# chrischoy/DeepGlobalRegistration

Measured on NVIDIA H100. Metric: scan_pairs_per_sec, higher is better.
Workload: dtype f32

## Files before the change

deepglobalregistration_b200/csrc/knn_tc.cu:

```cuda
#include <algorithm>

#include "common.cuh"
#include "tc_common.cuh"

namespace {

using namespace tc;

constexpr int kRows = 128;
constexpr int kTileBytes = kRows * 128;
constexpr int kTileFloats = kTileBytes / 4;
constexpr int kConsumerWarps = 8;
constexpr int kThreads = kConsumerWarps * 32 + 128;
constexpr int kQueue = 256;
constexpr float kInf = __builtin_huge_valf();

template <int C>
struct KnnCfg {
  static constexpr int kChunks = C / 32;
  static constexpr int kStages = C == 32 ? 4 : 3;
  static constexpr int kOpBytes = kChunks * kTileBytes;
  static constexpr size_t kSmem = 1024 + (size_t)(2 + kStages) * kOpBytes + kStages * kRows * 4 +
                                  kConsumerWarps * (kQueue + 16) * 8 + (2 * kStages + 4) * 8 + 16;
};

struct KnnWs {
  float* a_img;
  float* b_img;
  float* na2;
  unsigned* rowmin;
  float* nbh;
  float* bmax;
};
inline int64_t up4(int64_t x) { return (x + 3) & ~(int64_t)3; }
inline int64_t ceil_tiles(int64_t n) { return (n + kRows - 1) / kRows; }
void ws_offsets(int64_t n0, int64_t n1, int c, int64_t (&o)[7]) {
  const int64_t tile = (int64_t)(c / 32) * kTileFloats;
  o[0] = 0;
  o[1] = o[0] + ceil_tiles(n0) * tile;
  o[2] = o[1] + ceil_tiles(n1) * tile;
  o[3] = o[2] + up4(n0);
  o[4] = o[3] + up4(n0);
  o[5] = o[4] + ceil_tiles(n1) * kRows;
  o[6] = o[5] + up4(ceil_tiles(n1));
}
KnnWs carve_ws(float* ws, int64_t n0, int64_t n1, int c) {
  int64_t o[7];
  ws_offsets(n0, n1, c, o);
  return KnnWs{ws + o[0], ws + o[1], ws + o[2], reinterpret_cast<unsigned*>(ws + o[3]), ws + o[4], ws + o[5]};
}

__device__ __forceinline__ float knn_error_bound(float na, float nb) {
  return (0.0009765625f * 1.25f + 4e-5f) * na * nb + 1e-6f * (na + nb) * (na + nb) + 1e-7f;
}

template <int C>
__global__ void __launch_bounds__(kRows * 8)
knn_prep_kernel(const float* __restrict__ f0, int n0, const float* __restrict__ f1, int n1, int row_tiles, KnnWs w,
                unsigned long long* __restrict__ packed) {
  constexpr int kChunks = C / 32;
  const bool is_a = (int)blockIdx.x < row_tiles;
  const int tile = is_a ? blockIdx.x : blockIdx.x - row_tiles;
  const float* f = is_a ? f0 : f1;
  const int n = is_a ? n0 : n1;
  const int r = threadIdx.x >> 3, sub = threadIdx.x & 7;
  const int row = tile * kRows + r;
  const bool valid = row < n;
  float s = 0.f;
  if (valid)
    for (int k = sub; k < C; k += 8) {
      const float v = f[(size_t)row * C + k];
      s = fmaf(v, v, s);
    }
  s += __shfl_xor_sync(0xffffffffu, s, 1);
  s += __shfl_xor_sync(0xffffffffu, s, 2);
  s += __shfl_xor_sync(0xffffffffu, s, 4);
  float* img = (is_a ? w.a_img : w.b_img) + (size_t)tile * kChunks * kTileFloats;
#pragma unroll
  for (int ch = 0; ch < kChunks; ++ch) {
    float4 v = make_float4(0.f, 0.f, 0.f, 0.f);
    if (valid) v = __ldg(reinterpret_cast<const float4*>(f + (size_t)row * C + ch * 32 + sub * 4));
    v.x = tf32_round(v.x); v.y = tf32_round(v.y); v.z = tf32_round(v.z); v.w = tf32_round(v.w);
    *reinterpret_cast<float4*>(img + ch * kTileFloats + r * 32 + ((sub ^ (r & 7)) << 2)) = v;
  }
  if (is_a) {
    if (valid && sub == 0) {
      w.na2[row] = s;
      w.rowmin[row] = 0x7f800000u;
      packed[row] = ~0ull;
    }
    return;
  }
  if (sub == 0) w.nbh[row] = valid ? 0.5f * s : kInf;
  __shared__ float wmax[kRows * 8 / 32];
  float m = valid ? s : 0.f;
  m = fmaxf(m, __shfl_xor_sync(0xffffffffu, m, 8));
  m = fmaxf(m, __shfl_xor_sync(0xffffffffu, m, 16));
  if ((threadIdx.x & 31) == 0) wmax[threadIdx.x >> 5] = m;
  __syncthreads();
  if (threadIdx.x < 32) {
    m = wmax[threadIdx.x];
#pragma unroll
    for (int d = 16; d > 0; d >>= 1) m = fmaxf(m, __shfl_xor_sync(0xffffffffu, m, d));
    if (threadIdx.x == 0) w.bmax[tile] = m;
  }
}

template <int C>
__device__ __forceinline__ unsigned long long knn_exact_key(const float* __restrict__ f0, const float* __restrict__ f1,
                                                            int gi, int j) {
  const float4* a = reinterpret_cast<const float4*>(f0 + (size_t)gi * C);
  const float4* b = reinterpret_cast<const float4*>(f1 + (size_t)j * C);
  float d2 = 0.f;
#pragma unroll
  for (int k = 0; k < C / 4; ++k) {
    const float4 x = __ldg(a + k), y = __ldg(b + k);
    float df = x.x - y.x; d2 = fmaf(df, df, d2);
    df = x.y - y.y; d2 = fmaf(df, df, d2);
    df = x.z - y.z; d2 = fmaf(df, df, d2);
    df = x.w - y.w; d2 = fmaf(df, df, d2);
  }
  return ((unsigned long long)__float_as_uint(sqrtf(d2 + 1e-7f)) << 32) | (unsigned)j;
}

struct Item {
  int rt, ct0, ct1;
};
__device__ __forceinline__ Item item_at(long long k, long long k_end, int col_tiles) {
  Item it;
  it.rt = (int)(k / col_tiles);
  it.ct0 = (int)(k - (long long)it.rt * col_tiles);
  it.ct1 = (int)min((long long)col_tiles, it.ct0 + (k_end - k));
  return it;
}

template <int C, int PASS>
__global__ void __launch_bounds__(kThreads, 1)
knn_sweep_kernel(const float* __restrict__ f0, int n0, const float* __restrict__ f1, int row_tiles, int col_tiles,
                 KnnWs w, unsigned long long* __restrict__ packed) {
  using K = KnnCfg<C>;
  constexpr int kStages = K::kStages, kOpBytes = K::kOpBytes;
  extern __shared__ __align__(16) unsigned char smem_dyn[];
  unsigned char* a_buf = reinterpret_cast<unsigned char*>((reinterpret_cast<uintptr_t>(smem_dyn) + 1023) &
                                                          ~(uintptr_t)1023);
  unsigned char* b_buf = a_buf + 2 * kOpBytes;
  float* nb_buf = reinterpret_cast<float*>(b_buf + kStages * kOpBytes);
  unsigned long long* queue = reinterpret_cast<unsigned long long*>(nb_buf + kStages * kRows);
  unsigned long long* best = queue + kConsumerWarps * kQueue;
  uint64_t* bars = reinterpret_cast<uint64_t*>(best + kConsumerWarps * 16);
  const uint32_t full0 = smem_u32(bars), empty0 = full0 + 8 * kStages;
  const uint32_t a_full0 = empty0 + 8 * kStages, a_empty0 = a_full0 + 16;
  float* nbmax_sh = reinterpret_cast<float*>(bars + 2 * kStages + 4);

  const int t = threadIdx.x, warp = __shfl_sync(0xffffffffu, t >> 5, 0), lane = t & 31;
  const long long total = (long long)row_tiles * col_tiles;
  const long long k_begin = total * blockIdx.x / gridDim.x, k_end = total * (blockIdx.x + 1) / gridDim.x;

  if (t == 0) {
    for (int s = 0; s < kStages; ++s) {
      mbar_init(full0 + 8 * s, 1);
      mbar_init(empty0 + 8 * s, kConsumerWarps);
    }
    for (int p = 0; p < 2; ++p) {
      mbar_init(a_full0 + 8 * p, 1);
      mbar_init(a_empty0 + 8 * p, kConsumerWarps);
    }
    asm volatile("fence.mbarrier_init.release.cluster;" ::: "memory");
  }
  if (PASS == 2 && warp == 0) {
    float m = 0.f;
    for (int i = lane; i < col_tiles; i += 32) m = fmaxf(m, w.bmax[i]);
#pragma unroll
    for (int d = 16; d > 0; d >>= 1) m = fmaxf(m, __shfl_xor_sync(0xffffffffu, m, d));
    if (lane == 0) *nbmax_sh = m;
  }
  if (PASS == 2 && t < kConsumerWarps * 16) best[t] = ~0ull;
  __syncthreads();

  if (warp >= kConsumerWarps) {
    asm volatile("setmaxnreg.dec.sync.aligned.u32 40;");
    if (warp == kConsumerWarps && lane == 0) {
      long long kt = 0;
      int it = 0;
      for (long long k = k_begin; k < k_end; ++it) {
        const Item item = item_at(k, k_end, col_tiles);
        const int p = it & 1;
        if (it >= 2) mbar_wait(a_empty0 + 8 * p, ((it >> 1) - 1) & 1);
        mbar_arrive_expect_tx(a_full0 + 8 * p, kOpBytes);
        bulk_g2s(smem_u32(a_buf + p * kOpBytes), w.a_img + (size_t)item.rt * (kOpBytes / 4), kOpBytes, a_full0 + 8 * p);
        for (int ct = item.ct0; ct < item.ct1; ++ct, ++kt) {
          const int s = (int)(kt % kStages);
          if (kt >= kStages) mbar_wait(empty0 + 8 * s, (uint32_t)((kt / kStages - 1) & 1));
          mbar_arrive_expect_tx(full0 + 8 * s, kOpBytes + kRows * 4);
          bulk_g2s(smem_u32(b_buf + s * kOpBytes), w.b_img + (size_t)ct * (kOpBytes / 4), kOpBytes, full0 + 8 * s);
          bulk_g2s(smem_u32(nb_buf + s * kRows), w.nbh + (size_t)ct * kRows, kRows * 4, full0 + 8 * s);
        }
        k += item.ct1 - item.ct0;
      }
    }
    return;
  }

  asm volatile("setmaxnreg.inc.sync.aligned.u32 232;");
  const int wg = warp >> 2;
  const int rw = lane >> 2;
  const int row_in_tile = wg * 64 + (warp & 3) * 16;
  const float nb_root = PASS == 2 ? sqrtf(*nbmax_sh) : 0.f;
  unsigned long long* q = queue + warp * kQueue;
  unsigned long long* bw = best + warp * 16;
  int qn = 0;

  auto drain = [&](int row0) {
    __syncwarp();
    for (int b = 0; b < qn; b += 32)
      if (b + lane < qn) {
        const unsigned long long e = q[b + lane];
        const int r = (int)(e >> 32), j = (int)(unsigned)e;
        atomicMin(bw + r, knn_exact_key<C>(f0, f1, row0 + r, j));
      }
    qn = 0;
    __syncwarp();
  };

  long long kt = 0;
  int it = 0;
  for (long long k = k_begin; k < k_end; ++it) {
    const Item item = item_at(k, k_end, col_tiles);
    const int p = it & 1;
    const int row0 = item.rt * kRows + row_in_tile;
    int gi[2];
    float th[2], rmin[2][2];
#pragma unroll
    for (int h = 0; h < 2; ++h) {
      gi[h] = row0 + rw + 8 * h;
      th[h] = -kInf;
      if (PASS == 2 && gi[h] < n0) {
        const float na2 = w.na2[gi[h]];
        const float e = knn_error_bound(sqrtf(na2), nb_root);
        th[h] = 0.5f * (__uint_as_float(w.rowmin[gi[h]]) + 4.f * e - na2);
      }
      rmin[h][0] = rmin[h][1] = kInf;
    }
    mbar_wait(a_full0 + 8 * p, (it >> 1) & 1);
    const uint32_t a_s = smem_u32(a_buf + p * kOpBytes) + wg * (kTileBytes / 2);

    auto issue = [&](float(&acc)[64], long long kq) {
      const int s = (int)(kq % kStages);
      mbar_wait(full0 + 8 * s, (uint32_t)((kq / kStages) & 1));
      const uint32_t b_s = smem_u32(b_buf + s * kOpBytes);
      wgmma_fence();
#pragma unroll
      for (int ch = 0; ch < K::kChunks; ++ch)
#pragma unroll
        for (int ks = 0; ks < 4; ++ks)
          Wgmma<128, false>::mma(acc, wgmma_desc(a_s + ch * kTileBytes + ks * 32),
                                 wgmma_desc(b_s + ch * kTileBytes + ks * 32), (ch | ks) != 0);
      wgmma_commit();
    };
    auto epilogue = [&](float(&acc)[64], long long kq, int ct) {
      fence_acc(acc);
      const int s = (int)(kq % kStages);
      const float* nbs = nb_buf + s * kRows + 2 * (lane & 3);
      float tmin[2][2] = {{kInf, kInf}, {kInf, kInf}};
#pragma unroll
      for (int i = 0; i < kRows / 8; ++i) {
        const float2 nb = *reinterpret_cast<const float2*>(nbs + 8 * i);
#pragma unroll
        for (int h = 0; h < 2; ++h)
          tmin[h][i & 1] = fminf(tmin[h][i & 1], fminf(nb.x - acc[4 * i + 2 * h], nb.y - acc[4 * i + 2 * h + 1]));
      }
      if (PASS == 1) {
#pragma unroll
        for (int h = 0; h < 2; ++h) {
          rmin[h][0] = fminf(rmin[h][0], tmin[h][0]);
          rmin[h][1] = fminf(rmin[h][1], tmin[h][1]);
        }
      } else if (__any_sync(0xffffffffu, fminf(tmin[0][0], tmin[0][1]) <= th[0] ||
                                             fminf(tmin[1][0], tmin[1][1]) <= th[1])) {
        unsigned long long mask = 0;
#pragma unroll
        for (int i = 0; i < kRows / 8; ++i) {
          const float2 nb = *reinterpret_cast<const float2*>(nbs + 8 * i);
#pragma unroll
          for (int h = 0; h < 2; ++h)
#pragma unroll
            for (int e = 0; e < 2; ++e)
              if ((e ? nb.y : nb.x) - acc[4 * i + 2 * h + e] <= th[h]) mask |= 1ull << (4 * i + 2 * h + e);
        }
        const int cnt = __popcll(mask);
        int pos = cnt;
#pragma unroll
        for (int d = 1; d < 32; d <<= 1) {
          const int y = __shfl_up_sync(0xffffffffu, pos, d);
          if (lane >= d) pos += y;
        }
        const int total = __shfl_sync(0xffffffffu, pos, 31);
        pos -= cnt;
        if (qn + total > kQueue) drain(row0);
        for (int base = 0; base < total; base += kQueue) {
          unsigned long long m = mask;
          for (int idx = pos; m != 0; ++idx, m &= m - 1) {
            const int b = __ffsll((long long)m) - 1;
            if (idx >= base && idx < base + kQueue)
              q[qn + idx - base] = ((unsigned long long)(rw + 8 * ((b >> 1) & 1)) << 32) |
                                   (unsigned)(ct * kRows + 8 * (b >> 2) + 2 * (lane & 3) + (b & 1));
          }
          qn += min(kQueue, total - base);
          if (base + kQueue < total) drain(row0);
        }
      }
      __syncwarp();
      if (lane == 0) mbar_arrive(empty0 + 8 * s);
    };

    float acc0[64], acc1[64];
    const int n = item.ct1 - item.ct0;
    for (int i = 0; i < n; i += 2) {
      issue(acc0, kt + i);
      if (i + 1 < n) {
        issue(acc1, kt + i + 1);
        wgmma_wait<1>();
      } else {
        wgmma_wait<0>();
      }
      epilogue(acc0, kt + i, item.ct0 + i);
      if (i + 1 == n) break;
      wgmma_wait<0>();
      epilogue(acc1, kt + i + 1, item.ct0 + i + 1);
    }
    wgmma_wait<0>();
    __syncwarp();
    if (lane == 0) mbar_arrive(a_empty0 + 8 * p);
    kt += n;
    k += n;

    if (PASS == 1) {
#pragma unroll
      for (int h = 0; h < 2; ++h) {
        float m = fminf(rmin[h][0], rmin[h][1]);
        m = fminf(m, __shfl_xor_sync(0xffffffffu, m, 1));
        m = fminf(m, __shfl_xor_sync(0xffffffffu, m, 2));
        if (gi[h] < n0 && (lane & 3) == 0)
          atomicMin(w.rowmin + gi[h], __float_as_uint(fmaxf(fmaf(2.f, m, w.na2[gi[h]]), 0.f)));
      }
    } else {
      if (qn > 0) drain(row0);
      if (lane < 16) {
        const unsigned long long v = bw[lane];
        if (v != ~0ull && row0 + lane < n0) atomicMin(packed + row0 + lane, v);
        bw[lane] = ~0ull;
      }
      __syncwarp();
    }
  }
}

__global__ void knn_tc_unpack_kernel(const unsigned long long* __restrict__ packed, int64_t n,
                                     int32_t* __restrict__ idx, float* __restrict__ dist) {
  int64_t i = (int64_t)blockIdx.x * blockDim.x + threadIdx.x;
  if (i >= n) return;
  unsigned long long p = packed[i];
  idx[i] = (int32_t)(p & 0xffffffffu);
  if (dist != nullptr) dist[i] = __uint_as_float((unsigned)(p >> 32));
}

template <int C>
int32_t launch_knn_tc(const float* f0, int64_t n0, const float* f1, int64_t n1, const KnnWs& w,
                      unsigned long long* packed, cudaStream_t st) {
  constexpr size_t smem = KnnCfg<C>::kSmem;
  DGR_ENSURE_SMEM((knn_sweep_kernel<C, 1>), smem);
  DGR_ENSURE_SMEM((knn_sweep_kernel<C, 2>), smem);
  int dev = 0, sms = 0, per_sm1 = 0, per_sm2 = 0;
  DGR_CUDA_CHECK(cudaGetDevice(&dev));
  DGR_CUDA_CHECK(cudaDeviceGetAttribute(&sms, cudaDevAttrMultiProcessorCount, dev));
  DGR_CUDA_CHECK(cudaOccupancyMaxActiveBlocksPerMultiprocessor(&per_sm1, knn_sweep_kernel<C, 1>, kThreads, smem));
  DGR_CUDA_CHECK(cudaOccupancyMaxActiveBlocksPerMultiprocessor(&per_sm2, knn_sweep_kernel<C, 2>, kThreads, smem));
  const int row_tiles = (int)ceil_tiles(n0), col_tiles = (int)ceil_tiles(n1);
  const long long total = (long long)row_tiles * col_tiles;
  const int grid = (int)std::min<long long>(total, (long long)sms * std::max(1, std::min(per_sm1, per_sm2)));
  knn_prep_kernel<C><<<row_tiles + col_tiles, kRows * 8, 0, st>>>(f0, (int)n0, f1, (int)n1, row_tiles, w, packed);
  knn_sweep_kernel<C, 1><<<grid, kThreads, smem, st>>>(f0, (int)n0, f1, row_tiles, col_tiles, w, packed);
  knn_sweep_kernel<C, 2><<<grid, kThreads, smem, st>>>(f0, (int)n0, f1, row_tiles, col_tiles, w, packed);
  return DGR_OK;
}

}

extern "C" {

int64_t dgr_knn_tc_ws_elems(int64_t n0, int64_t n1, int32_t c) {
  int64_t o[7];
  ws_offsets(n0, n1, c, o);
  return o[6];
}

int32_t dgr_knn_tc_supported(int32_t c) { return (c == 32 || c == 64) ? 1 : 0; }

int32_t dgr_knn_top1_tc(const float* f0, int64_t n0, const float* f1, int64_t n1, int32_t c,
                        uint64_t* packed_ws, float* ws, int32_t* idx, float* dist, void* stream) {
  DGR_ARG_CHECK(dgr_knn_tc_supported(c), "channel count not supported by the tensor-core kNN");
  DGR_ARG_CHECK(n1 >= 1 || n0 == 0, "F1 must not be empty");
  DGR_ARG_CHECK(n0 < (1ll << 31) && n1 < (1ll << 31), "too many rows");
  DGR_ARG_CHECK(((uintptr_t)ws & 15) == 0, "workspace must be 16-byte aligned");
  if (n0 == 0) return DGR_OK;
  cudaStream_t st = (cudaStream_t)stream;
  const KnnWs w = carve_ws(ws, n0, n1, c);
  unsigned long long* packed = reinterpret_cast<unsigned long long*>(packed_ws);
  int32_t rc = (c == 32) ? launch_knn_tc<32>(f0, n0, f1, n1, w, packed, st)
                         : launch_knn_tc<64>(f0, n0, f1, n1, w, packed, st);
  if (rc != DGR_OK) return rc;
  knn_tc_unpack_kernel<<<dgr_blocks(n0, 256), 256, 0, st>>>(packed, n0, idx, dist);
  dgr_note_launches(4);
  DGR_LAUNCH_CHECK();
  return DGR_OK;
}

}
```

deepglobalregistration_b200/csrc/tc_common.cuh:

```cuda
#pragma once
#include <cuda_fp16.h>
#include <cuda_runtime.h>
#include <stdint.h>

#include "wgmma.cuh"

namespace tc {

__device__ __forceinline__ uint32_t smem_u32(const void* p) {
  return (uint32_t)__cvta_generic_to_shared(p);
}
__device__ __forceinline__ void mbar_init(uint32_t bar, uint32_t count) {
  asm volatile("mbarrier.init.shared::cta.b64 [%0], %1;" ::"r"(bar), "r"(count) : "memory");
}
__device__ __forceinline__ bool mbar_try_wait(uint32_t bar, uint32_t parity) {
  uint32_t ok;
  asm volatile(
      "{\n\t.reg .pred p;\n\t"
      "mbarrier.try_wait.parity.shared::cta.b64 p, [%1], %2;\n\t"
      "selp.u32 %0, 1, 0, p;\n\t}"
      : "=r"(ok)
      : "r"(bar), "r"(parity)
      : "memory");
  return ok != 0;
}
__device__ __forceinline__ void mbar_wait(uint32_t bar, uint32_t parity) {
  while (!mbar_try_wait(bar, parity)) {
  }
}
__device__ __forceinline__ void mbar_arrive(uint32_t bar) {
  asm volatile("mbarrier.arrive.shared::cta.b64 _, [%0];" ::"r"(bar) : "memory");
}
__device__ __forceinline__ void mbar_arrive_expect_tx(uint32_t bar, uint32_t bytes) {
  asm volatile("mbarrier.arrive.expect_tx.shared::cta.b64 _, [%0], %1;" ::"r"(bar), "r"(bytes) : "memory");
}
__device__ __forceinline__ void fence_proxy_async() {
  asm volatile("fence.proxy.async.shared::cta;" ::: "memory");
}
__device__ __forceinline__ void bulk_g2s(uint32_t dst_smem, const void* src, uint32_t bytes, uint32_t bar) {
  asm volatile("cp.async.bulk.shared::cluster.global.mbarrier::complete_tx::bytes [%0], [%1], %2, [%3];" ::"r"(
                   dst_smem),
               "l"(src), "r"(bytes), "r"(bar)
               : "memory");
}

__device__ __forceinline__ uint64_t wgmma_desc(uint32_t smem_addr) {
  uint64_t d = 0;
  d |= (uint64_t)((smem_addr & 0x3FFFFu) >> 4);
  d |= (uint64_t)1 << 16;
  d |= (uint64_t)(1024 >> 4) << 32;
  d |= (uint64_t)1 << 62;
  return d;
}
__device__ __forceinline__ void wgmma_fence() { asm volatile("wgmma.fence.sync.aligned;" ::: "memory"); }
__device__ __forceinline__ void wgmma_commit() { asm volatile("wgmma.commit_group.sync.aligned;" ::: "memory"); }
template <int kPending>
__device__ __forceinline__ void wgmma_wait() {
  asm volatile("wgmma.wait_group.sync.aligned %0;" ::"n"(kPending) : "memory");
}
template <int R>
__device__ __forceinline__ void fence_acc(float (&d)[R]) {
#pragma unroll
  for (int i = 0; i < R; ++i) asm volatile("" : "+f"(d[i])::"memory");
}

__device__ __forceinline__ void red_add_v2(float* addr, float a, float b) {
  asm volatile("red.global.add.v2.f32 [%0], {%1, %2};" ::"l"(addr), "f"(a), "f"(b) : "memory");
}
__device__ __forceinline__ void red_add_v4(float* addr, float a, float b, float c, float d) {
  asm volatile("red.global.add.v4.f32 [%0], {%1, %2, %3, %4};" ::"l"(addr), "f"(a), "f"(b), "f"(c), "f"(d)
               : "memory");
}
__device__ __forceinline__ float tf32_round(float x) {
  uint32_t r;
  asm("cvt.rna.tf32.f32 %0, %1;" : "=r"(r) : "f"(x));
  return __uint_as_float(r);
}

__device__ __forceinline__ void split_store(float4 v, unsigned char* hi_tile, unsigned char* lo_tile, uint32_t off) {
  float4 h, l;
  h.x = tf32_round(v.x); h.y = tf32_round(v.y); h.z = tf32_round(v.z); h.w = tf32_round(v.w);
  l.x = v.x - h.x; l.y = v.y - h.y; l.z = v.z - h.z; l.w = v.w - h.w;
  *reinterpret_cast<float4*>(hi_tile + off) = h;
  *reinterpret_cast<float4*>(lo_tile + off) = l;
}

__device__ __forceinline__ void split_store_f16(float4 a, float4 b, float sx, unsigned char* hi_tile,
                                                unsigned char* lo_tile, uint32_t off) {
  const float x[8] = {a.x * sx, a.y * sx, a.z * sx, a.w * sx, b.x * sx, b.y * sx, b.z * sx, b.w * sx};
  uint32_t h[4], l[4];
#pragma unroll
  for (int i = 0; i < 4; ++i) {
    const __half2 hh = __floats2half2_rn(x[2 * i], x[2 * i + 1]);
    const float2 hf = __half22float2(hh);
    const __half2 ll = __floats2half2_rn(x[2 * i] - hf.x, x[2 * i + 1] - hf.y);
    h[i] = *reinterpret_cast<const uint32_t*>(&hh);
    l[i] = *reinterpret_cast<const uint32_t*>(&ll);
  }
  *reinterpret_cast<uint4*>(hi_tile + off) = make_uint4(h[0], h[1], h[2], h[3]);
  *reinterpret_cast<uint4*>(lo_tile + off) = make_uint4(l[0], l[1], l[2], l[3]);
}
__device__ __forceinline__ float f16_scale_for(float amax) {
  const uint32_t b = __float_as_uint(amax);
  const int e = (int)((b >> 23) & 255u);
  if (e == 0 || e == 255) return 1.f;
  int se = 14 - (e - 127) + 127;
  se = se < 1 ? 1 : (se > 254 ? 254 : se);
  return __uint_as_float((uint32_t)se << 23);
}

template <int N, bool kF16, int kPasses>
__device__ __forceinline__ void mma_chunk(float (&d)[N / 2], uint32_t a_hi, uint32_t a_lo, uint32_t b_hi,
                                          uint32_t b_lo) {
#pragma unroll
  for (int ks = 0; ks < 4; ++ks) {
    const uint32_t ko = ks * 32;
    const uint64_t dbh = wgmma_desc(b_hi + ko);
    Wgmma<N, kF16>::mma(d, wgmma_desc(a_hi + ko), dbh);
    if (kPasses == 3) {
      Wgmma<N, kF16>::mma(d, wgmma_desc(a_lo + ko), dbh);
      Wgmma<N, kF16>::mma(d, wgmma_desc(a_hi + ko), wgmma_desc(b_lo + ko));
    }
  }
}

}
```

deepglobalregistration_b200/csrc/wgmma.cuh:

```cuda
#pragma once
#include <stdint.h>

namespace tc {

template <int N, bool kF16>
struct Wgmma;

template <>
struct Wgmma<32, false> {
  __device__ __forceinline__ static void mma(float (&d)[16], uint64_t a, uint64_t b) {
    asm volatile(
        "{\n\t.reg .pred p;\n\tsetp.ne.b32 p, %18, 0;\n\t"
        "wgmma.mma_async.sync.aligned.m64n32k8.f32.tf32.tf32 "
        "{%0, %1, %2, %3, %4, %5, %6, %7, %8, %9, %10, %11, %12, %13, %14, %15}, %16, %17, p, 1, 1;\n\t}"
        : "+f"(d[0]), "+f"(d[1]), "+f"(d[2]), "+f"(d[3]), "+f"(d[4]), "+f"(d[5]), "+f"(d[6]), "+f"(d[7]),
          "+f"(d[8]), "+f"(d[9]), "+f"(d[10]), "+f"(d[11]), "+f"(d[12]), "+f"(d[13]), "+f"(d[14]), "+f"(d[15])
        : "l"(a), "l"(b), "r"(1));
  }
};

template <>
struct Wgmma<64, false> {
  __device__ __forceinline__ static void mma(float (&d)[32], uint64_t a, uint64_t b) {
    asm volatile(
        "{\n\t.reg .pred p;\n\tsetp.ne.b32 p, %34, 0;\n\t"
        "wgmma.mma_async.sync.aligned.m64n64k8.f32.tf32.tf32 "
        "{%0, %1, %2, %3, %4, %5, %6, %7, %8, %9, %10, %11, %12, %13, %14, %15, "
        "%16, %17, %18, %19, %20, %21, %22, %23, %24, %25, %26, %27, %28, %29, %30, %31}, %32, %33, p, 1, 1;\n\t}"
        : "+f"(d[0]), "+f"(d[1]), "+f"(d[2]), "+f"(d[3]), "+f"(d[4]), "+f"(d[5]), "+f"(d[6]), "+f"(d[7]),
          "+f"(d[8]), "+f"(d[9]), "+f"(d[10]), "+f"(d[11]), "+f"(d[12]), "+f"(d[13]), "+f"(d[14]), "+f"(d[15]),
          "+f"(d[16]), "+f"(d[17]), "+f"(d[18]), "+f"(d[19]), "+f"(d[20]), "+f"(d[21]), "+f"(d[22]), "+f"(d[23]),
          "+f"(d[24]), "+f"(d[25]), "+f"(d[26]), "+f"(d[27]), "+f"(d[28]), "+f"(d[29]), "+f"(d[30]), "+f"(d[31])
        : "l"(a), "l"(b), "r"(1));
  }
};

template <>
struct Wgmma<128, false> {
  __device__ __forceinline__ static void mma(float (&d)[64], uint64_t a, uint64_t b, int scale_d = 1) {
    asm volatile(
        "{\n\t.reg .pred p;\n\tsetp.ne.b32 p, %66, 0;\n\t"
        "wgmma.mma_async.sync.aligned.m64n128k8.f32.tf32.tf32 "
        "{%0, %1, %2, %3, %4, %5, %6, %7, %8, %9, %10, %11, %12, %13, %14, %15, "
        "%16, %17, %18, %19, %20, %21, %22, %23, %24, %25, %26, %27, %28, %29, %30, %31, "
        "%32, %33, %34, %35, %36, %37, %38, %39, %40, %41, %42, %43, %44, %45, %46, %47, "
        "%48, %49, %50, %51, %52, %53, %54, %55, %56, %57, %58, %59, %60, %61, %62, %63}, %64, %65, p, 1, 1;\n\t}"
        : "+f"(d[0]), "+f"(d[1]), "+f"(d[2]), "+f"(d[3]), "+f"(d[4]), "+f"(d[5]), "+f"(d[6]), "+f"(d[7]),
          "+f"(d[8]), "+f"(d[9]), "+f"(d[10]), "+f"(d[11]), "+f"(d[12]), "+f"(d[13]), "+f"(d[14]), "+f"(d[15]),
          "+f"(d[16]), "+f"(d[17]), "+f"(d[18]), "+f"(d[19]), "+f"(d[20]), "+f"(d[21]), "+f"(d[22]), "+f"(d[23]),
          "+f"(d[24]), "+f"(d[25]), "+f"(d[26]), "+f"(d[27]), "+f"(d[28]), "+f"(d[29]), "+f"(d[30]), "+f"(d[31]),
          "+f"(d[32]), "+f"(d[33]), "+f"(d[34]), "+f"(d[35]), "+f"(d[36]), "+f"(d[37]), "+f"(d[38]), "+f"(d[39]),
          "+f"(d[40]), "+f"(d[41]), "+f"(d[42]), "+f"(d[43]), "+f"(d[44]), "+f"(d[45]), "+f"(d[46]), "+f"(d[47]),
          "+f"(d[48]), "+f"(d[49]), "+f"(d[50]), "+f"(d[51]), "+f"(d[52]), "+f"(d[53]), "+f"(d[54]), "+f"(d[55]),
          "+f"(d[56]), "+f"(d[57]), "+f"(d[58]), "+f"(d[59]), "+f"(d[60]), "+f"(d[61]), "+f"(d[62]), "+f"(d[63])
        : "l"(a), "l"(b), "r"(scale_d));
  }
};

template <>
struct Wgmma<256, false> {
  __device__ __forceinline__ static void mma(float (&d)[128], uint64_t a, uint64_t b) {
    asm volatile(
        "{\n\t.reg .pred p;\n\tsetp.ne.b32 p, %130, 0;\n\t"
        "wgmma.mma_async.sync.aligned.m64n256k8.f32.tf32.tf32 "
        "{%0, %1, %2, %3, %4, %5, %6, %7, %8, %9, %10, %11, %12, %13, %14, %15, "
        "%16, %17, %18, %19, %20, %21, %22, %23, %24, %25, %26, %27, %28, %29, %30, %31, "
        "%32, %33, %34, %35, %36, %37, %38, %39, %40, %41, %42, %43, %44, %45, %46, %47, "
        "%48, %49, %50, %51, %52, %53, %54, %55, %56, %57, %58, %59, %60, %61, %62, %63, "
        "%64, %65, %66, %67, %68, %69, %70, %71, %72, %73, %74, %75, %76, %77, %78, %79, "
        "%80, %81, %82, %83, %84, %85, %86, %87, %88, %89, %90, %91, %92, %93, %94, %95, "
        "%96, %97, %98, %99, %100, %101, %102, %103, %104, %105, %106, %107, %108, %109, %110, %111, "
        "%112, %113, %114, %115, %116, %117, %118, %119, %120, %121, %122, %123, %124, %125, %126, %127}, %128, %129, p, 1, 1;\n\t}"
        : "+f"(d[0]), "+f"(d[1]), "+f"(d[2]), "+f"(d[3]), "+f"(d[4]), "+f"(d[5]), "+f"(d[6]), "+f"(d[7]),
          "+f"(d[8]), "+f"(d[9]), "+f"(d[10]), "+f"(d[11]), "+f"(d[12]), "+f"(d[13]), "+f"(d[14]), "+f"(d[15]),
          "+f"(d[16]), "+f"(d[17]), "+f"(d[18]), "+f"(d[19]), "+f"(d[20]), "+f"(d[21]), "+f"(d[22]), "+f"(d[23]),
          "+f"(d[24]), "+f"(d[25]), "+f"(d[26]), "+f"(d[27]), "+f"(d[28]), "+f"(d[29]), "+f"(d[30]), "+f"(d[31]),
          "+f"(d[32]), "+f"(d[33]), "+f"(d[34]), "+f"(d[35]), "+f"(d[36]), "+f"(d[37]), "+f"(d[38]), "+f"(d[39]),
          "+f"(d[40]), "+f"(d[41]), "+f"(d[42]), "+f"(d[43]), "+f"(d[44]), "+f"(d[45]), "+f"(d[46]), "+f"(d[47]),
          "+f"(d[48]), "+f"(d[49]), "+f"(d[50]), "+f"(d[51]), "+f"(d[52]), "+f"(d[53]), "+f"(d[54]), "+f"(d[55]),
          "+f"(d[56]), "+f"(d[57]), "+f"(d[58]), "+f"(d[59]), "+f"(d[60]), "+f"(d[61]), "+f"(d[62]), "+f"(d[63]),
          "+f"(d[64]), "+f"(d[65]), "+f"(d[66]), "+f"(d[67]), "+f"(d[68]), "+f"(d[69]), "+f"(d[70]), "+f"(d[71]),
          "+f"(d[72]), "+f"(d[73]), "+f"(d[74]), "+f"(d[75]), "+f"(d[76]), "+f"(d[77]), "+f"(d[78]), "+f"(d[79]),
          "+f"(d[80]), "+f"(d[81]), "+f"(d[82]), "+f"(d[83]), "+f"(d[84]), "+f"(d[85]), "+f"(d[86]), "+f"(d[87]),
          "+f"(d[88]), "+f"(d[89]), "+f"(d[90]), "+f"(d[91]), "+f"(d[92]), "+f"(d[93]), "+f"(d[94]), "+f"(d[95]),
          "+f"(d[96]), "+f"(d[97]), "+f"(d[98]), "+f"(d[99]), "+f"(d[100]), "+f"(d[101]), "+f"(d[102]), "+f"(d[103]),
          "+f"(d[104]), "+f"(d[105]), "+f"(d[106]), "+f"(d[107]), "+f"(d[108]), "+f"(d[109]), "+f"(d[110]), "+f"(d[111]),
          "+f"(d[112]), "+f"(d[113]), "+f"(d[114]), "+f"(d[115]), "+f"(d[116]), "+f"(d[117]), "+f"(d[118]), "+f"(d[119]),
          "+f"(d[120]), "+f"(d[121]), "+f"(d[122]), "+f"(d[123]), "+f"(d[124]), "+f"(d[125]), "+f"(d[126]), "+f"(d[127])
        : "l"(a), "l"(b), "r"(1));
  }
};

template <>
struct Wgmma<32, true> {
  __device__ __forceinline__ static void mma(float (&d)[16], uint64_t a, uint64_t b) {
    asm volatile(
        "{\n\t.reg .pred p;\n\tsetp.ne.b32 p, %18, 0;\n\t"
        "wgmma.mma_async.sync.aligned.m64n32k16.f32.f16.f16 "
        "{%0, %1, %2, %3, %4, %5, %6, %7, %8, %9, %10, %11, %12, %13, %14, %15}, %16, %17, p, 1, 1, 0, 0;\n\t}"
        : "+f"(d[0]), "+f"(d[1]), "+f"(d[2]), "+f"(d[3]), "+f"(d[4]), "+f"(d[5]), "+f"(d[6]), "+f"(d[7]),
          "+f"(d[8]), "+f"(d[9]), "+f"(d[10]), "+f"(d[11]), "+f"(d[12]), "+f"(d[13]), "+f"(d[14]), "+f"(d[15])
        : "l"(a), "l"(b), "r"(1));
  }
};

template <>
struct Wgmma<64, true> {
  __device__ __forceinline__ static void mma(float (&d)[32], uint64_t a, uint64_t b) {
    asm volatile(
        "{\n\t.reg .pred p;\n\tsetp.ne.b32 p, %34, 0;\n\t"
        "wgmma.mma_async.sync.aligned.m64n64k16.f32.f16.f16 "
        "{%0, %1, %2, %3, %4, %5, %6, %7, %8, %9, %10, %11, %12, %13, %14, %15, "
        "%16, %17, %18, %19, %20, %21, %22, %23, %24, %25, %26, %27, %28, %29, %30, %31}, %32, %33, p, 1, 1, 0, 0;\n\t}"
        : "+f"(d[0]), "+f"(d[1]), "+f"(d[2]), "+f"(d[3]), "+f"(d[4]), "+f"(d[5]), "+f"(d[6]), "+f"(d[7]),
          "+f"(d[8]), "+f"(d[9]), "+f"(d[10]), "+f"(d[11]), "+f"(d[12]), "+f"(d[13]), "+f"(d[14]), "+f"(d[15]),
          "+f"(d[16]), "+f"(d[17]), "+f"(d[18]), "+f"(d[19]), "+f"(d[20]), "+f"(d[21]), "+f"(d[22]), "+f"(d[23]),
          "+f"(d[24]), "+f"(d[25]), "+f"(d[26]), "+f"(d[27]), "+f"(d[28]), "+f"(d[29]), "+f"(d[30]), "+f"(d[31])
        : "l"(a), "l"(b), "r"(1));
  }
};

template <>
struct Wgmma<128, true> {
  __device__ __forceinline__ static void mma(float (&d)[64], uint64_t a, uint64_t b) {
    asm volatile(
        "{\n\t.reg .pred p;\n\tsetp.ne.b32 p, %66, 0;\n\t"
        "wgmma.mma_async.sync.aligned.m64n128k16.f32.f16.f16 "
        "{%0, %1, %2, %3, %4, %5, %6, %7, %8, %9, %10, %11, %12, %13, %14, %15, "
        "%16, %17, %18, %19, %20, %21, %22, %23, %24, %25, %26, %27, %28, %29, %30, %31, "
        "%32, %33, %34, %35, %36, %37, %38, %39, %40, %41, %42, %43, %44, %45, %46, %47, "
        "%48, %49, %50, %51, %52, %53, %54, %55, %56, %57, %58, %59, %60, %61, %62, %63}, %64, %65, p, 1, 1, 0, 0;\n\t}"
        : "+f"(d[0]), "+f"(d[1]), "+f"(d[2]), "+f"(d[3]), "+f"(d[4]), "+f"(d[5]), "+f"(d[6]), "+f"(d[7]),
          "+f"(d[8]), "+f"(d[9]), "+f"(d[10]), "+f"(d[11]), "+f"(d[12]), "+f"(d[13]), "+f"(d[14]), "+f"(d[15]),
          "+f"(d[16]), "+f"(d[17]), "+f"(d[18]), "+f"(d[19]), "+f"(d[20]), "+f"(d[21]), "+f"(d[22]), "+f"(d[23]),
          "+f"(d[24]), "+f"(d[25]), "+f"(d[26]), "+f"(d[27]), "+f"(d[28]), "+f"(d[29]), "+f"(d[30]), "+f"(d[31]),
          "+f"(d[32]), "+f"(d[33]), "+f"(d[34]), "+f"(d[35]), "+f"(d[36]), "+f"(d[37]), "+f"(d[38]), "+f"(d[39]),
          "+f"(d[40]), "+f"(d[41]), "+f"(d[42]), "+f"(d[43]), "+f"(d[44]), "+f"(d[45]), "+f"(d[46]), "+f"(d[47]),
          "+f"(d[48]), "+f"(d[49]), "+f"(d[50]), "+f"(d[51]), "+f"(d[52]), "+f"(d[53]), "+f"(d[54]), "+f"(d[55]),
          "+f"(d[56]), "+f"(d[57]), "+f"(d[58]), "+f"(d[59]), "+f"(d[60]), "+f"(d[61]), "+f"(d[62]), "+f"(d[63])
        : "l"(a), "l"(b), "r"(1));
  }
};

template <>
struct Wgmma<256, true> {
  __device__ __forceinline__ static void mma(float (&d)[128], uint64_t a, uint64_t b) {
    asm volatile(
        "{\n\t.reg .pred p;\n\tsetp.ne.b32 p, %130, 0;\n\t"
        "wgmma.mma_async.sync.aligned.m64n256k16.f32.f16.f16 "
        "{%0, %1, %2, %3, %4, %5, %6, %7, %8, %9, %10, %11, %12, %13, %14, %15, "
        "%16, %17, %18, %19, %20, %21, %22, %23, %24, %25, %26, %27, %28, %29, %30, %31, "
        "%32, %33, %34, %35, %36, %37, %38, %39, %40, %41, %42, %43, %44, %45, %46, %47, "
        "%48, %49, %50, %51, %52, %53, %54, %55, %56, %57, %58, %59, %60, %61, %62, %63, "
        "%64, %65, %66, %67, %68, %69, %70, %71, %72, %73, %74, %75, %76, %77, %78, %79, "
        "%80, %81, %82, %83, %84, %85, %86, %87, %88, %89, %90, %91, %92, %93, %94, %95, "
        "%96, %97, %98, %99, %100, %101, %102, %103, %104, %105, %106, %107, %108, %109, %110, %111, "
        "%112, %113, %114, %115, %116, %117, %118, %119, %120, %121, %122, %123, %124, %125, %126, %127}, %128, %129, p, 1, 1, 0, 0;\n\t}"
        : "+f"(d[0]), "+f"(d[1]), "+f"(d[2]), "+f"(d[3]), "+f"(d[4]), "+f"(d[5]), "+f"(d[6]), "+f"(d[7]),
          "+f"(d[8]), "+f"(d[9]), "+f"(d[10]), "+f"(d[11]), "+f"(d[12]), "+f"(d[13]), "+f"(d[14]), "+f"(d[15]),
          "+f"(d[16]), "+f"(d[17]), "+f"(d[18]), "+f"(d[19]), "+f"(d[20]), "+f"(d[21]), "+f"(d[22]), "+f"(d[23]),
          "+f"(d[24]), "+f"(d[25]), "+f"(d[26]), "+f"(d[27]), "+f"(d[28]), "+f"(d[29]), "+f"(d[30]), "+f"(d[31]),
          "+f"(d[32]), "+f"(d[33]), "+f"(d[34]), "+f"(d[35]), "+f"(d[36]), "+f"(d[37]), "+f"(d[38]), "+f"(d[39]),
          "+f"(d[40]), "+f"(d[41]), "+f"(d[42]), "+f"(d[43]), "+f"(d[44]), "+f"(d[45]), "+f"(d[46]), "+f"(d[47]),
          "+f"(d[48]), "+f"(d[49]), "+f"(d[50]), "+f"(d[51]), "+f"(d[52]), "+f"(d[53]), "+f"(d[54]), "+f"(d[55]),
          "+f"(d[56]), "+f"(d[57]), "+f"(d[58]), "+f"(d[59]), "+f"(d[60]), "+f"(d[61]), "+f"(d[62]), "+f"(d[63]),
          "+f"(d[64]), "+f"(d[65]), "+f"(d[66]), "+f"(d[67]), "+f"(d[68]), "+f"(d[69]), "+f"(d[70]), "+f"(d[71]),
          "+f"(d[72]), "+f"(d[73]), "+f"(d[74]), "+f"(d[75]), "+f"(d[76]), "+f"(d[77]), "+f"(d[78]), "+f"(d[79]),
          "+f"(d[80]), "+f"(d[81]), "+f"(d[82]), "+f"(d[83]), "+f"(d[84]), "+f"(d[85]), "+f"(d[86]), "+f"(d[87]),
          "+f"(d[88]), "+f"(d[89]), "+f"(d[90]), "+f"(d[91]), "+f"(d[92]), "+f"(d[93]), "+f"(d[94]), "+f"(d[95]),
          "+f"(d[96]), "+f"(d[97]), "+f"(d[98]), "+f"(d[99]), "+f"(d[100]), "+f"(d[101]), "+f"(d[102]), "+f"(d[103]),
          "+f"(d[104]), "+f"(d[105]), "+f"(d[106]), "+f"(d[107]), "+f"(d[108]), "+f"(d[109]), "+f"(d[110]), "+f"(d[111]),
          "+f"(d[112]), "+f"(d[113]), "+f"(d[114]), "+f"(d[115]), "+f"(d[116]), "+f"(d[117]), "+f"(d[118]), "+f"(d[119]),
          "+f"(d[120]), "+f"(d[121]), "+f"(d[122]), "+f"(d[123]), "+f"(d[124]), "+f"(d[125]), "+f"(d[126]), "+f"(d[127])
        : "l"(a), "l"(b), "r"(1));
  }
};

}
```

Measured before the change: 81.75.

## Switch KNN tensor-core sweep from TF32 to scaled FP16 operands

Replaces the TF32 operand images with per-cloud scaled FP16 images. The scale comes from a global abs-max found by a new norms kernel, and a separate image kernel writes the swizzled half-precision tiles. Operand bytes are halved, pipeline stages are doubled, and the wgmma instruction count per tile drops. The exactness filter's error bound is widened to cover FP16 quantisation, which may admit more candidates to the exact refinement pass. The change also adds an extra kernel launch plus a memset, a 4-tile grouped issue/epilogue loop, and neighbour-norm prefetch into registers.

```diff
diff --git a/deepglobalregistration_b200/csrc/knn_tc.cu b/deepglobalregistration_b200/csrc/knn_tc.cu
--- a/deepglobalregistration_b200/csrc/knn_tc.cu
+++ b/deepglobalregistration_b200/csrc/knn_tc.cu
@@ -8,34 +8,38 @@
 using namespace tc;
 
 constexpr int kRows = 128;
-constexpr int kTileBytes = kRows * 128;
-constexpr int kTileFloats = kTileBytes / 4;
 constexpr int kConsumerWarps = 8;
 constexpr int kThreads = kConsumerWarps * 32 + 128;
 constexpr int kQueue = 256;
+constexpr int kGroup = 4;
 constexpr float kInf = __builtin_huge_valf();
 
 template <int C>
 struct KnnCfg {
-  static constexpr int kChunks = C / 32;
-  static constexpr int kStages = C == 32 ? 4 : 3;
-  static constexpr int kOpBytes = kChunks * kTileBytes;
+  static constexpr int kRowBytes = C * 2;
+  static constexpr int kOpBytes = kRows * kRowBytes;
+  static constexpr int kStages = C == 32 ? 8 : 6;
   static constexpr size_t kSmem = 1024 + (size_t)(2 + kStages) * kOpBytes + kStages * kRows * 4 +
                                   kConsumerWarps * (kQueue + 16) * 8 + (2 * kStages + 4) * 8 + 16;
 };
+template <int C>
+__device__ __forceinline__ uint64_t op_desc(uint32_t smem_addr) {
+  return C == 32 ? wgmma_desc_sw64(smem_addr) : wgmma_desc(smem_addr);
+}
 
 struct KnnWs {
-  float* a_img;
-  float* b_img;
+  unsigned char* a_img;
+  unsigned char* b_img;
   float* na2;
   unsigned* rowmin;
   float* nbh;
   float* bmax;
+  float* amax;
 };
 inline int64_t up4(int64_t x) { return (x + 3) & ~(int64_t)3; }
 inline int64_t ceil_tiles(int64_t n) { return (n + kRows - 1) / kRows; }
-void ws_offsets(int64_t n0, int64_t n1, int c, int64_t (&o)[7]) {
-  const int64_t tile = (int64_t)(c / 32) * kTileFloats;
+void ws_offsets(int64_t n0, int64_t n1, int c, int64_t (&o)[8]) {
+  const int64_t tile = (int64_t)kRows * c / 2;
   o[0] = 0;
   o[1] = o[0] + ceil_tiles(n0) * tile;
   o[2] = o[1] + ceil_tiles(n1) * tile;
@@ -43,22 +47,30 @@
   o[4] = o[3] + up4(n0);
   o[5] = o[4] + ceil_tiles(n1) * kRows;
   o[6] = o[5] + up4(ceil_tiles(n1));
+  o[7] = o[6] + 4;
 }
 KnnWs carve_ws(float* ws, int64_t n0, int64_t n1, int c) {
-  int64_t o[7];
+  int64_t o[8];
   ws_offsets(n0, n1, c, o);
-  return KnnWs{ws + o[0], ws + o[1], ws + o[2], reinterpret_cast<unsigned*>(ws + o[3]), ws + o[4], ws + o[5]};
-}
-
-__device__ __forceinline__ float knn_error_bound(float na, float nb) {
-  return (0.0009765625f * 1.25f + 4e-5f) * na * nb + 1e-6f * (na + nb) * (na + nb) + 1e-7f;
+  return KnnWs{reinterpret_cast<unsigned char*>(ws + o[0]), reinterpret_cast<unsigned char*>(ws + o[1]), ws + o[2],
+               reinterpret_cast<unsigned*>(ws + o[3]), ws + o[4], ws + o[5], ws + o[6]};
+}
+
+__device__ __forceinline__ float knn_scale(float amax) {
+  return fminf(fmaxf(f16_scale_for(amax), 0x1p-62f), 0x1p62f);
+}
+
+template <int C>
+__device__ __forceinline__ float knn_error_bound(float na, float nb, float alpha, float beta) {
+  constexpr float kRootC = C == 32 ? 5.6568543f : 8.f;
+  return (0.0009765625f * 1.25f + 4e-5f) * na * nb + 1.01f * kRootC * (alpha * nb + beta * na + kRootC * alpha * beta) +
+         1e-6f * (na + nb) * (na + nb) + 1e-7f;
 }
 
 template <int C>
 __global__ void __launch_bounds__(kRows * 8)
-knn_prep_kernel(const float* __restrict__ f0, int n0, const float* __restrict__ f1, int n1, int row_tiles, KnnWs w,
-                unsigned long long* __restrict__ packed) {
-  constexpr int kChunks = C / 32;
+knn_norms_kernel(const float* __restrict__ f0, int n0, const float* __restrict__ f1, int n1, int row_tiles, KnnWs w,
+                 unsigned long long* __restrict__ packed) {
   const bool is_a = (int)blockIdx.x < row_tiles;
   const int tile = is_a ? blockIdx.x : blockIdx.x - row_tiles;
   const float* f = is_a ? f0 : f1;
@@ -66,44 +78,75 @@
   const int r = threadIdx.x >> 3, sub = threadIdx.x & 7;
   const int row = tile * kRows + r;
   const bool valid = row < n;
-  float s = 0.f;
+  float s = 0.f, am = 0.f;
   if (valid)
     for (int k = sub; k < C; k += 8) {
       const float v = f[(size_t)row * C + k];
       s = fmaf(v, v, s);
+      am = fmaxf(am, fabsf(v));
     }
   s += __shfl_xor_sync(0xffffffffu, s, 1);
   s += __shfl_xor_sync(0xffffffffu, s, 2);
   s += __shfl_xor_sync(0xffffffffu, s, 4);
-  float* img = (is_a ? w.a_img : w.b_img) + (size_t)tile * kChunks * kTileFloats;
-#pragma unroll
-  for (int ch = 0; ch < kChunks; ++ch) {
-    float4 v = make_float4(0.f, 0.f, 0.f, 0.f);
-    if (valid) v = __ldg(reinterpret_cast<const float4*>(f + (size_t)row * C + ch * 32 + sub * 4));
-    v.x = tf32_round(v.x); v.y = tf32_round(v.y); v.z = tf32_round(v.z); v.w = tf32_round(v.w);
-    *reinterpret_cast<float4*>(img + ch * kTileFloats + r * 32 + ((sub ^ (r & 7)) << 2)) = v;
-  }
-  if (is_a) {
-    if (valid && sub == 0) {
-      w.na2[row] = s;
-      w.rowmin[row] = 0x7f800000u;
-      packed[row] = ~0ull;
-    }
-    return;
-  }
-  if (sub == 0) w.nbh[row] = valid ? 0.5f * s : kInf;
-  __shared__ float wmax[kRows * 8 / 32];
+  if (is_a && valid && sub == 0) {
+    w.na2[row] = s;
+    w.rowmin[row] = 0x7f800000u;
+    packed[row] = ~0ull;
+  }
+  if (!is_a && sub == 0) w.nbh[row] = valid ? 0.5f * s : kInf;
+  __shared__ float wmax[2][kRows * 8 / 32];
   float m = valid ? s : 0.f;
+#pragma unroll
+  for (int d = 1; d < 32; d <<= 1) am = fmaxf(am, __shfl_xor_sync(0xffffffffu, am, d));
   m = fmaxf(m, __shfl_xor_sync(0xffffffffu, m, 8));
   m = fmaxf(m, __shfl_xor_sync(0xffffffffu, m, 16));
-  if ((threadIdx.x & 31) == 0) wmax[threadIdx.x >> 5] = m;
+  if ((threadIdx.x & 31) == 0) {
+    wmax[0][threadIdx.x >> 5] = m;
+    wmax[1][threadIdx.x >> 5] = am;
+  }
   __syncthreads();
   if (threadIdx.x < 32) {
-    m = wmax[threadIdx.x];
-#pragma unroll
-    for (int d = 16; d > 0; d >>= 1) m = fmaxf(m, __shfl_xor_sync(0xffffffffu, m, d));
-    if (threadIdx.x == 0) w.bmax[tile] = m;
-  }
+    m = wmax[0][threadIdx.x];
+    am = wmax[1][threadIdx.x];
+#pragma unroll
+    for (int d = 16; d > 0; d >>= 1) {
+      m = fmaxf(m, __shfl_xor_sync(0xffffffffu, m, d));
+      am = fmaxf(am, __shfl_xor_sync(0xffffffffu, am, d));
+    }
+    if (threadIdx.x == 0) {
+      if (!is_a) w.bmax[tile] = m;
+      atomicMax(reinterpret_cast<unsigned*>(w.amax) + (is_a ? 0 : 1), __float_as_uint(am));
+    }
+  }
+}
+
+template <int C>
+__global__ void __launch_bounds__(kRows * 8)
+knn_image_kernel(const float* __restrict__ f0, int n0, const float* __restrict__ f1, int n1, int row_tiles, KnnWs w) {
+  constexpr int kRowBytes = KnnCfg<C>::kRowBytes, kPieces = kRowBytes / 16;
+  const bool is_a = (int)blockIdx.x < row_tiles;
+  const int tile = is_a ? blockIdx.x : blockIdx.x - row_tiles;
+  const float* f = is_a ? f0 : f1;
+  const int n = is_a ? n0 : n1;
+  const int r = threadIdx.x >> 3, sub = threadIdx.x & 7;
+  const int row = tile * kRows + r;
+  if (sub >= kPieces) return;
+  const float sx = knn_scale(w.amax[is_a ? 0 : 1]);
+  float4 v[2] = {make_float4(0.f, 0.f, 0.f, 0.f), make_float4(0.f, 0.f, 0.f, 0.f)};
+  if (row < n) {
+    v[0] = __ldg(reinterpret_cast<const float4*>(f + (size_t)row * C + sub * 8));
+    v[1] = __ldg(reinterpret_cast<const float4*>(f + (size_t)row * C + sub * 8 + 4));
+  }
+  uint32_t h[4];
+#pragma unroll
+  for (int i = 0; i < 2; ++i) {
+    const __half2 lo = __floats2half2_rn(v[i].x * sx, v[i].y * sx), hi = __floats2half2_rn(v[i].z * sx, v[i].w * sx);
+    h[2 * i] = *reinterpret_cast<const uint32_t*>(&lo);
+    h[2 * i + 1] = *reinterpret_cast<const uint32_t*>(&hi);
+  }
+  const int piece = sub ^ ((r * kRowBytes >> 7) & (kPieces - 1));
+  unsigned char* img = (is_a ? w.a_img : w.b_img) + (size_t)tile * KnnCfg<C>::kOpBytes;
+  *reinterpret_cast<uint4*>(img + r * kRowBytes + piece * 16) = make_uint4(h[0], h[1], h[2], h[3]);
 }
 
 template <int C>
@@ -121,6 +164,12 @@
     df = x.w - y.w; d2 = fmaf(df, df, d2);
   }
   return ((unsigned long long)__float_as_uint(sqrtf(d2 + 1e-7f)) << 32) | (unsigned)j;
+}
+
+__device__ __forceinline__ float2 lds_f2(uint32_t addr) {
+  float2 v;
+  asm volatile("ld.shared.v2.f32 {%0, %1}, [%2];" : "=f"(v.x), "=f"(v.y) : "r"(addr) : "memory");
+  return v;
 }
 
 struct Item {
@@ -187,12 +236,12 @@
         const int p = it & 1;
         if (it >= 2) mbar_wait(a_empty0 + 8 * p, ((it >> 1) - 1) & 1);
         mbar_arrive_expect_tx(a_full0 + 8 * p, kOpBytes);
-        bulk_g2s(smem_u32(a_buf + p * kOpBytes), w.a_img + (size_t)item.rt * (kOpBytes / 4), kOpBytes, a_full0 + 8 * p);
+        bulk_g2s(smem_u32(a_buf + p * kOpBytes), w.a_img + (size_t)item.rt * kOpBytes, kOpBytes, a_full0 + 8 * p);
         for (int ct = item.ct0; ct < item.ct1; ++ct, ++kt) {
           const int s = (int)(kt % kStages);
           if (kt >= kStages) mbar_wait(empty0 + 8 * s, (uint32_t)((kt / kStages - 1) & 1));
           mbar_arrive_expect_tx(full0 + 8 * s, kOpBytes + kRows * 4);
-          bulk_g2s(smem_u32(b_buf + s * kOpBytes), w.b_img + (size_t)ct * (kOpBytes / 4), kOpBytes, full0 + 8 * s);
+          bulk_g2s(smem_u32(b_buf + s * kOpBytes), w.b_img + (size_t)ct * kOpBytes, kOpBytes, full0 + 8 * s);
           bulk_g2s(smem_u32(nb_buf + s * kRows), w.nbh + (size_t)ct * kRows, kRows * 4, full0 + 8 * s);
         }
         k += item.ct1 - item.ct0;
@@ -206,6 +255,8 @@
   const int rw = lane >> 2;
   const int row_in_tile = wg * 64 + (warp & 3) * 16;
   const float nb_root = PASS == 2 ? sqrtf(*nbmax_sh) : 0.f;
+  const float sa = knn_scale(w.amax[0]), sb = knn_scale(w.amax[1]);
+  const float inv = 1.f / (sa * sb), alpha = 0x1p-25f / sa, beta = 0x1p-25f / sb;
   unsigned long long* q = queue + warp * kQueue;
   unsigned long long* bw = best + warp * 16;
   int qn = 0;
@@ -236,13 +287,13 @@
       th[h] = -kInf;
       if (PASS == 2 && gi[h] < n0) {
         const float na2 = w.na2[gi[h]];
-        const float e = knn_error_bound(sqrtf(na2), nb_root);
+        const float e = knn_error_bound<C>(sqrtf(na2), nb_root, alpha, beta);
         th[h] = 0.5f * (__uint_as_float(w.rowmin[gi[h]]) + 4.f * e - na2);
       }
       rmin[h][0] = rmin[h][1] = kInf;
     }
     mbar_wait(a_full0 + 8 * p, (it >> 1) & 1);
-    const uint32_t a_s = smem_u32(a_buf + p * kOpBytes) + wg * (kTileBytes / 2);
+    const uint32_t a_s = smem_u32(a_buf + p * kOpBytes) + wg * (kOpBytes / 2);
 
     auto issue = [&](float(&acc)[64], long long kq) {
       const int s = (int)(kq % kStages);
@@ -250,24 +301,26 @@
       const uint32_t b_s = smem_u32(b_buf + s * kOpBytes);
       wgmma_fence();
 #pragma unroll
-      for (int ch = 0; ch < K::kChunks; ++ch)
-#pragma unroll
-        for (int ks = 0; ks < 4; ++ks)
-          Wgmma<128, false>::mma(acc, wgmma_desc(a_s + ch * kTileBytes + ks * 32),
-                                 wgmma_desc(b_s + ch * kTileBytes + ks * 32), (ch | ks) != 0);
+      for (int ks = 0; ks < C / 16; ++ks)
+        Wgmma<128, true>::mma(acc, op_desc<C>(a_s + ks * 32), op_desc<C>(b_s + ks * 32), ks != 0);
       wgmma_commit();
     };
-    auto epilogue = [&](float(&acc)[64], long long kq, int ct) {
+    auto load_nb = [&](float2(&nb)[kRows / 8], long long kq) {
+      const uint32_t nbs = smem_u32(nb_buf + (int)(kq % kStages) * kRows + 2 * (lane & 3));
+#pragma unroll
+      for (int i = 0; i < kRows / 8; ++i) nb[i] = lds_f2(nbs + 32 * i);
+    };
+    auto epilogue = [&](float(&acc)[64], const float2(&nbv)[kRows / 8], long long kq, int ct) {
       fence_acc(acc);
       const int s = (int)(kq % kStages);
-      const float* nbs = nb_buf + s * kRows + 2 * (lane & 3);
       float tmin[2][2] = {{kInf, kInf}, {kInf, kInf}};
 #pragma unroll
       for (int i = 0; i < kRows / 8; ++i) {
-        const float2 nb = *reinterpret_cast<const float2*>(nbs + 8 * i);
+        const float2 nb = nbv[i];
 #pragma unroll
         for (int h = 0; h < 2; ++h)
-          tmin[h][i & 1] = fminf(tmin[h][i & 1], fminf(nb.x - acc[4 * i + 2 * h], nb.y - acc[4 * i + 2 * h + 1]));
+          tmin[h][i & 1] = fminf(tmin[h][i & 1], fminf(fmaf(-inv, acc[4 * i + 2 * h], nb.x),
+                                                       fmaf(-inv, acc[4 * i + 2 * h + 1], nb.y)));
       }
       if (PASS == 1) {
 #pragma unroll
@@ -280,12 +333,12 @@
         unsigned long long mask = 0;
 #pragma unroll
         for (int i = 0; i < kRows / 8; ++i) {
-          const float2 nb = *reinterpret_cast<const float2*>(nbs + 8 * i);
+          const float2 nb = nbv[i];
 #pragma unroll
           for (int h = 0; h < 2; ++h)
 #pragma unroll
             for (int e = 0; e < 2; ++e)
-              if ((e ? nb.y : nb.x) - acc[4 * i + 2 * h + e] <= th[h]) mask |= 1ull << (4 * i + 2 * h + e);
+              if (fmaf(-inv, acc[4 * i + 2 * h + e], e ? nb.y : nb.x) <= th[h]) mask |= 1ull << (4 * i + 2 * h + e);
         }
         const int cnt = __popcll(mask);
         int pos = cnt;
@@ -314,19 +367,36 @@
     };
 
     float acc0[64], acc1[64];
+    float2 nbv[kRows / 8];
     const int n = item.ct1 - item.ct0;
-    for (int i = 0; i < n; i += 2) {
+    int i = 0;
+    for (; i + kGroup <= n; i += kGroup) {
       issue(acc0, kt + i);
+      issue(acc1, kt + i + 1);
+#pragma unroll
+      for (int u = 0; u < kGroup; ++u) {
+        float(&acc)[64] = (u & 1) ? acc1 : acc0;
+        load_nb(nbv, kt + i + u);
+        if (u + 1 < kGroup) wgmma_wait<1>();
+        else wgmma_wait<0>();
+        epilogue(acc, nbv, kt + i + u, item.ct0 + i + u);
+        if (u + 2 < kGroup) issue(acc, kt + i + u + 2);
+      }
+    }
+    for (; i < n; i += 2) {
+      issue(acc0, kt + i);
+      load_nb(nbv, kt + i);
       if (i + 1 < n) {
         issue(acc1, kt + i + 1);
         wgmma_wait<1>();
       } else {
         wgmma_wait<0>();
       }
-      epilogue(acc0, kt + i, item.ct0 + i);
+      epilogue(acc0, nbv, kt + i, item.ct0 + i);
       if (i + 1 == n) break;
+      load_nb(nbv, kt + i + 1);
       wgmma_wait<0>();
-      epilogue(acc1, kt + i + 1, item.ct0 + i + 1);
+      epilogue(acc1, nbv, kt + i + 1, item.ct0 + i + 1);
     }
     wgmma_wait<0>();
     __syncwarp();
@@ -378,7 +448,9 @@
   const int row_tiles = (int)ceil_tiles(n0), col_tiles = (int)ceil_tiles(n1);
   const long long total = (long long)row_tiles * col_tiles;
   const int grid = (int)std::min<long long>(total, (long long)sms * std::max(1, std::min(per_sm1, per_sm2)));
-  knn_prep_kernel<C><<<row_tiles + col_tiles, kRows * 8, 0, st>>>(f0, (int)n0, f1, (int)n1, row_tiles, w, packed);
+  DGR_CUDA_CHECK(cudaMemsetAsync(w.amax, 0, 2 * sizeof(float), st));
+  knn_norms_kernel<C><<<row_tiles + col_tiles, kRows * 8, 0, st>>>(f0, (int)n0, f1, (int)n1, row_tiles, w, packed);
+  knn_image_kernel<C><<<row_tiles + col_tiles, kRows * 8, 0, st>>>(f0, (int)n0, f1, (int)n1, row_tiles, w);
   knn_sweep_kernel<C, 1><<<grid, kThreads, smem, st>>>(f0, (int)n0, f1, row_tiles, col_tiles, w, packed);
   knn_sweep_kernel<C, 2><<<grid, kThreads, smem, st>>>(f0, (int)n0, f1, row_tiles, col_tiles, w, packed);
   return DGR_OK;
@@ -389,9 +461,9 @@
 extern "C" {
 
 int64_t dgr_knn_tc_ws_elems(int64_t n0, int64_t n1, int32_t c) {
-  int64_t o[7];
+  int64_t o[8];
   ws_offsets(n0, n1, c, o);
-  return o[6];
+  return o[7];
 }
 
 int32_t dgr_knn_tc_supported(int32_t c) { return (c == 32 || c == 64) ? 1 : 0; }
@@ -410,7 +482,7 @@
                          : launch_knn_tc<64>(f0, n0, f1, n1, w, packed, st);
   if (rc != DGR_OK) return rc;
   knn_tc_unpack_kernel<<<dgr_blocks(n0, 256), 256, 0, st>>>(packed, n0, idx, dist);
-  dgr_note_launches(4);
+  dgr_note_launches(5);
   DGR_LAUNCH_CHECK();
   return DGR_OK;
 }
diff --git a/deepglobalregistration_b200/csrc/tc_common.cuh b/deepglobalregistration_b200/csrc/tc_common.cuh
--- a/deepglobalregistration_b200/csrc/tc_common.cuh
+++ b/deepglobalregistration_b200/csrc/tc_common.cuh
@@ -50,6 +50,14 @@
   d |= (uint64_t)1 << 16;
   d |= (uint64_t)(1024 >> 4) << 32;
   d |= (uint64_t)1 << 62;
+  return d;
+}
+__device__ __forceinline__ uint64_t wgmma_desc_sw64(uint32_t smem_addr) {
+  uint64_t d = 0;
+  d |= (uint64_t)((smem_addr & 0x3FFFFu) >> 4);
+  d |= (uint64_t)1 << 16;
+  d |= (uint64_t)(512 >> 4) << 32;
+  d |= (uint64_t)2 << 62;
   return d;
 }
 __device__ __forceinline__ void wgmma_fence() { asm volatile("wgmma.fence.sync.aligned;" ::: "memory"); }
diff --git a/deepglobalregistration_b200/csrc/wgmma.cuh b/deepglobalregistration_b200/csrc/wgmma.cuh
--- a/deepglobalregistration_b200/csrc/wgmma.cuh
+++ b/deepglobalregistration_b200/csrc/wgmma.cuh
@@ -122,7 +122,7 @@
 
 template <>
 struct Wgmma<128, true> {
-  __device__ __forceinline__ static void mma(float (&d)[64], uint64_t a, uint64_t b) {
+  __device__ __forceinline__ static void mma(float (&d)[64], uint64_t a, uint64_t b, int scale_d = 1) {
     asm volatile(
         "{\n\t.reg .pred p;\n\tsetp.ne.b32 p, %66, 0;\n\t"
         "wgmma.mma_async.sync.aligned.m64n128k16.f32.f16.f16 "
@@ -138,7 +138,7 @@
           "+f"(d[40]), "+f"(d[41]), "+f"(d[42]), "+f"(d[43]), "+f"(d[44]), "+f"(d[45]), "+f"(d[46]), "+f"(d[47]),
           "+f"(d[48]), "+f"(d[49]), "+f"(d[50]), "+f"(d[51]), "+f"(d[52]), "+f"(d[53]), "+f"(d[54]), "+f"(d[55]),
           "+f"(d[56]), "+f"(d[57]), "+f"(d[58]), "+f"(d[59]), "+f"(d[60]), "+f"(d[61]), "+f"(d[62]), "+f"(d[63])
-        : "l"(a), "l"(b), "r"(1));
+        : "l"(a), "l"(b), "r"(scale_d));
   }
 };
 
```

Result: no change. 81.81 (median of 6 runs) (+0.1%).
